# Adoni5/mappy-rs

Measured on AMD Instinct MI355X. Metric: aligned Mbases/sec, ONT reads vs GRCh38 map-ont, 1/2/4/8 MI355X, higher is better.
Workload: dtype u8/int32 (+f32 chaining gap cost, f64 RMQ priority)

## Files before the change

mappy-rs_amd/csrc/mm355_dp.hip:

```cpp
#include <hip/hip_runtime.h>
#include <stdio.h>
#include <string.h>
#include <vector>
#include <mutex>
#include <condition_variable>
#include <algorithm>
#include "mm355_pipeline.h"
#include "mm355_dp.h"
#include "mm355_dpdomain.h"

#define WAVE 64
#define KSW_NEG_INF (-0x40000000)

struct EzState { int32_t max, max_q, max_t, mqe, mqe_t, mte, mte_q, score, zdropped, reach_end; };

__device__ inline int8_t I8(int v) { return (int8_t)v; }

__device__ __forceinline__ bool apply_zdrop(EzState &ez, int32_t H, int r, int t, int zdrop, int e2)
{
	if (H > ez.max) {
		ez.max = H, ez.max_t = t, ez.max_q = r - t;
	} else if (t >= ez.max_t && r - t >= ez.max_q) {
		int tl = t - ez.max_t, ql = (r - t) - ez.max_q, l;
		l = tl > ql? tl - ql : ql - tl;
// ... 221 lines not shown
			if (r - st0 == qlen - 1 && Hst0 > ez.mqe) ez.mqe = Hst0, ez.mqe_t = st0;
			if (apply_zdrop(ez, max_H, r, max_t, zdrop, e2)) break;
			if (r == qlen + tlen - 2 && en0 == tlen - 1) ez.score = H[tlen - 1];
		} else {
			if (r > 0) {
				if (last_H0_t >= st0 && last_H0_t <= en0 && last_H0_t + 1 >= st0 && last_H0_t + 1 <= en0) {
					int32_t d0 = SB(S[last_H0_t], 1);
					int32_t d1 = SB(S[last_H0_t + 1], 0);
					if (d0 > d1) H0 += d0;
					else H0 += d1, ++last_H0_t;
				} else if (last_H0_t >= st0 && last_H0_t <= en0) {
					H0 += SB(S[last_H0_t], 1);
				} else {
					++last_H0_t, H0 += SB(S[last_H0_t], 0);
				}
			} else H0 = (int32_t)SB(S[0], 1) - qe, last_H0_t = 0;
			if ((flag & EZ_APPROX_DROP) && apply_zdrop(ez, H0, r, last_H0_t, zdrop, e2)) break;
			if (r == qlen + tlen - 2 && en0 == tlen - 1) ez.score = H0;
		}
		last_st = st, last_en = en;
		DP_SYNC();
	}
	if (lane == 0) {
		int i0 = -1, j0 = -1;
		if (!ez.zdropped && !(flag & EZ_EXTZ_ONLY)) { i0 = tlen - 1; j0 = qlen - 1; }
		else if (!ez.zdropped && (flag & EZ_EXTZ_ONLY) && ez.mqe + end_bonus > ez.max) { ez.reach_end = 1; i0 = ez.mqe_t; j0 = qlen - 1; }
		else if (ez.max_t >= 0 && ez.max_q >= 0) { i0 = ez.max_t; j0 = ez.max_q; }
		mm355_dpres_t o;
		o.max = ez.max; o.zdropped = ez.zdropped; o.max_q = ez.max_q; o.max_t = ez.max_t; o.mqe = ez.mqe; o.mqe_t = ez.mqe_t;
		o.mte = ez.mte; o.mte_q = ez.mte_q; o.score = ez.score; o.reach_end = ez.reach_end;
		o.n_cigar = i0;
		o.cigar_off = j0;
		res[jid] = o;
		if (cells) atomicAdd((cls_base >= 0? cells_ctr + DP_CTR_SPREAD * (2 * (cls_base + (T > 4096) + (T > 12288)) + (approx_max? 0 : 1)) : cells_ctr) + (blockIdx.x & (DP_CTR_SPREAD - 1)), cells);
	}
}

#include "mm355_dpreg.h"
#include "mm355_dpmw.h"
#include "mm355_dprow.h"
#include "mm355_dpband.h"

__global__ __launch_bounds__(WAVE) void k_ksw_backtrack(const DpJobDev *jobs, const int32_t *job_ids, int n_jobs, const uint8_t *pbase, const uint8_t *pbase2, uint32_t *cigbase,
                                                        mm355_dpres_t *res, uint32_t *dense, unsigned long long *dense_ctr)
{
	const int t = blockIdx.x * WAVE + threadIdx.x;
	if (t >= n_jobs) return;
	const int jid = job_ids[t];
	const DpJobDev jb = jobs[jid];
	mm355_dpres_t o = res[jid];
	const int i0 = o.n_cigar, j0 = (int)o.cigar_off;
	int n_cigar = 0;
	uint32_t *cigar = cigbase + jb.cig_off;
	const int qlen = jb.qlen, tlen = jb.tlen;
	if (qlen > 0 && tlen > 0 && !jb.skip && (i0 >= 0 || j0 >= 0)) {
		int w = jb.w;
		if (w < 0) w = tlen > qlen? tlen : qlen;
		int n_col_ = qlen < tlen? qlen : tlen;
		n_col_ = ((n_col_ < w + 1? n_col_ : w + 1) + 15) / 16 + 1;
		const int n_col = n_col_ * 16;
		const uint8_t *p = (jb.pad & 4? pbase2 : pbase) + jb.p_off;
		const int lay = jb.pad & 3, dlo = jb.dlo;
		const int row_stride = lay == 2? jb.bw : (tlen + 15) / 16 * 16 + 16;
		int i = i0, j = j0, state = 0;
		uint32_t run_op = 0, run_len = 0;
#define BT_PUSH(op, len) do { if (run_len && run_op == (uint32_t)(op)) run_len += (uint32_t)(len); else { if (run_len) cigar[n_cigar++] = run_len << 4 | run_op; run_op = (uint32_t)(op); run_len = (uint32_t)(len); } } while (0)
		while (i >= 0 && j >= 0) {
			int force_state = -1, rr = i + j;
			int st = 0, en = tlen - 1;
			if (st < rr - qlen + 1) st = rr - qlen + 1;
			if (en > rr) en = rr;
			if (st < (rr - w + 1) >> 1) st = (rr - w + 1) >> 1;
			if (en > (rr + w) >> 1) en = (rr + w) >> 1;
			st = st / 16 * 16, en = (en + 16) / 16 * 16 - 1;
			uint32_t tmp;
			if (i < st) force_state = 2;
			if (i > en) force_state = 1;
			tmp = force_state < 0? (lay == 1? p[row_cell_off(j, i, row_stride)] : lay == 2? p[row_cell_off(j, min(max(i - j - dlo, 0), row_stride - 1), row_stride)] : p[(size_t)rr * n_col + i - st]) : 0;
			if (state == 0) state = tmp & 7;
			else if (!(tmp >> (state + 2) & 1)) state = 0;
			if (state == 0) state = tmp & 7;
			if (force_state >= 0) state = force_state;
			if (state == 0) { BT_PUSH(0, 1); --i; --j; }
			else if (state == 1 || state == 3) { BT_PUSH(2, 1); --i; }
			else { BT_PUSH(1, 1); --j; }
		}
		if (i >= 0) BT_PUSH(2, i + 1);
		if (j >= 0) BT_PUSH(1, j + 1);
		if (run_len) cigar[n_cigar++] = run_len << 4 | run_op;
#undef BT_PUSH
	}
	long long dst;
	{
		const int lane = threadIdx.x & 63;
		unsigned int inc = (unsigned int)n_cigar;
		for (int d = 1; d < 64; d <<= 1) { const unsigned int u = __shfl_up(inc, d); if (lane >= d) inc += u; }
		const int last = 63 - __builtin_clzll(__ballot(1));
		unsigned long long base = 0;
		if (lane == last) base = atomicAdd(dense_ctr, (unsigned long long)inc);
		base = __shfl(base, last);
		dst = (long long)(base + inc - (unsigned int)n_cigar);
	}
	if (jb.flag & EZ_REV_CIGAR) for (int k = 0; k < n_cigar; ++k) dense[dst + k] = cigar[k];
	else for (int k = 0; k < n_cigar; ++k) dense[dst + k] = cigar[n_cigar - 1 - k];
	o.n_cigar = n_cigar; o.cigar_off = dst;
	res[jid] = o;
}

__global__ __launch_bounds__(256) void k_dp_gather(DevIndex ix, const DpGather *g, int n_jobs, const uint8_t *rq, uint8_t *qbuf, uint8_t *tbuf)
{
	const int j = blockIdx.x;
	if (j >= n_jobs) return;
	const DpGather gj = g[j];
	for (int i = threadIdx.x; i < gj.qlen; i += 256) {
		const int src = gj.rev? gj.qlen - 1 - i : i;
		qbuf[gj.qoff + i] = rq[gj.q_src + src];
	}
	const uint64_t base = ix.seq_off[gj.rid] + (uint64_t)gj.t_st;
	__shared__ uint32_t s_first, s_cnt;
	if (threadIdx.x == 0) { uint32_t f = 0, n = 0; if (ix.n_nr) ref_window(ix, base, base + (uint64_t)(gj.tlen > 0? gj.tlen : 0), f, n); s_first = f; s_cnt = n; }
	__syncthreads();
	const uint32_t first = s_first, cnt = s_cnt;
	for (int i = threadIdx.x; i < gj.tlen; i += 256) {
		const int src = gj.rev? gj.tlen - 1 - i : i;
		tbuf[gj.toff + i] = (uint8_t)ref_code(ix, first, cnt, base + (uint64_t)src);
	}
}

__global__ __launch_bounds__(256) void k_read_codes(DevBatch bt, uint8_t *rq)
{
	const int r = blockIdx.x;
	const int len = bt.rlen[r];
	const int64_t off = bt.roff[r];
	for (int i = threadIdx.x; i < len; i += 256) {
		const int c = mm_nt4(bt.seq[off + i]);
		rq[2 * off + i] = (uint8_t)c;
		rq[2 * off + len + (len - 1 - i)] = (uint8_t)(c < 4? 3 - c : 4);
	}
}

static const DpKnobs &dp_knobs()
{
	static const DpKnobs kn = [] {
		auto on = [](const char *name) { const char *e = getenv(name); return !(e && atoi(e) == 0); };
		DpKnobs k;
		k.use_row = on("MM355_DP_ROW"); k.use_rowl = on("MM355_DP_ROWL"); k.use_regw = on("MM355_DP_REGW"); k.regw8 = on("MM355_DP_REGW8");
		k.use_band = on("MM355_DP_BAND");
		if (const char *e = getenv("MM355_DP_BAND_THR")) k.band_thr = atof(e);
		if (const char *e = getenv("MM355_DP_BAND_THR_HALF")) k.band_thr_half = atof(e);
		if (const char *e = getenv("MM355_DP_BAND_FORCE")) k.band_force = atoi(e);
		return k;
	}();
	return kn;
}

size_t mm355_dp_matrix_bytes(const mm355_mapopt_t *mo, const DpConst &dc, int qlen, int tlen, int w_in, int flag)
{
	return mm355_dp_plan_budget(mm355_dp_plan(dc, dp_knobs(), mo->max_sw_mat, qlen, tlen, w_in, flag));
}

__global__ void k_dp_patch(DpJobDev *jobs, const int32_t *ids, const DpJobDev *nj, int n) { const int i = blockIdx.x * blockDim.x + threadIdx.x; if (i < n) jobs[ids[i]] = nj[i]; }

struct DpLaunchArgs {
	DpConst dc; const DpJobDev *jobs; const uint8_t *d_q, *d_t; uint8_t *bt; mm355_dpres_t *res;
	int32_t *d_off; uint32_t *cig; uint64_t *d_S; int32_t *d_H; uint32_t *dense; unsigned long long *d_dense;
	int32_t *d_fail;
	unsigned long long *d_gcells;
	size_t regw_seq;
	size_t n_band2_right;
};
typedef int (*DpLauncher)(const DpLaunchArgs &a, hipStream_t st, const int32_t *ids, unsigned n, unsigned long long *cells);

typedef void (*DpKernel)(DpConst, const DpJobDev*, const int32_t*, int, const uint8_t*, const uint8_t*, uint8_t*, mm355_dpres_t*, unsigned long long*);
template <DpKernel K, int NT = 64>
static int launch(const DpLaunchArgs &a, hipStream_t st, const int32_t *ids, unsigned n, unsigned long long *cells)
{
	hipLaunchKernelGGL(K, dim3(n), dim3(NT), 0, st, a.dc, a.jobs, ids, (int)n, a.d_q, a.d_t, a.bt, a.res, cells);
	return 0;
}
template <int CLS>
static int launch_lds(const DpLaunchArgs &a, hipStream_t st, const int32_t *ids, unsigned n, unsigned long long *)
{
	const int cap = DP_CLASS_CAP[CLS];
	(void)hipFuncSetAttribute((const void*)k_ksw_extd2<512>, hipFuncAttributeMaxDynamicSharedMemorySize, DP_CLASS_CAP[DP_N_CLASS - 2] * 12);
	hipLaunchKernelGGL(k_ksw_extd2<512>, dim3(n), dim3(512), (size_t)cap * 12, st, a.dc, a.jobs, ids, (int)n, a.d_q, a.d_t, a.bt, a.d_off, a.cig, a.d_S, a.d_H, a.res,
	                   cap, a.d_gcells, a.dense, a.d_dense, 4);
	return 0;
}
static int launch_regw(const DpLaunchArgs &a, hipStream_t st, const int32_t *ids, unsigned n, unsigned long long *cells)
{
	if (!dp_knobs().regw8) return launch<k_ksw_regw>(a, st, ids, n, cells);
	if (a.regw_seq + 64 > 32768 && hipFuncSetAttribute((const void*)k_ksw_regw8, hipFuncAttributeMaxDynamicSharedMemorySize, MW_SEQ_MAX + 64) != hipSuccess) return MM355_EHIP;
	hipLaunchKernelGGL(k_ksw_regw8, dim3(n), dim3(MW_THREADS), a.regw_seq + 64, st, a.dc, a.jobs, ids, (int)n, a.d_q, a.d_t, a.bt, a.res, cells);
	return 0;
}
template <int NS>
static int launch_band(const DpLaunchArgs &a, hipStream_t st, const int32_t *ids, unsigned n, unsigned long long *cells)
{
	hipLaunchKernelGGL(k_ksw_band<NS>, dim3(n), dim3(64), 0, st, a.dc, a.jobs, ids, (int)n, a.d_q, a.d_t, a.bt, a.res, cells, a.d_fail);
	return 0;
}
static int launch_band2(const DpLaunchArgs &a, hipStream_t st, const int32_t *ids, unsigned n, unsigned long long *cells)
{
	const unsigned nr = (unsigned)a.n_band2_right, nl = n - nr;
	if (nr) hipLaunchKernelGGL(k_ksw_band2, dim3((nr + 1) / 2), dim3(64), 0, st, a.dc, a.jobs, ids, (int)nr, a.d_q, a.d_t, a.bt, a.res, cells, a.d_fail);
	if (nl) hipLaunchKernelGGL(k_ksw_band2, dim3((nl + 1) / 2), dim3(64), 0, st, a.dc, a.jobs, ids + nr, (int)nl, a.d_q, a.d_t, a.bt, a.res, cells, a.d_fail);
	return 0;
}

struct DpUnit { int g0, g1; DpLauncher launch; int stream; bool in_turn, join_at_once; };
static const DpUnit DP_UNITS[] = {
	{ DP_G_LDS + 2, DP_G_ROW2,      launch_lds<5>,                       5, false, false },
// ... 24 lines not shown
	std::mutex m; std::condition_variable cv; int busy = 0;
	void lock(int cap) { std::unique_lock<std::mutex> lk(m); cv.wait(lk, [&] { return busy < cap; }); ++busy; }
	void unlock() { { std::lock_guard<std::mutex> lk(m); --busy; } cv.notify_one(); }
};
struct TurnGuard { Turn *t = 0; void lock(Turn *x, int cap) { x->lock(cap); t = x; } void unlock() { if (t) { t->unlock(); t = 0; } } ~TurnGuard() { unlock(); } };

static int group_begin(mm355_ctx *c, int g, hipStream_t gst)
{
	if (c->dp_ev[g] == 0) HIPCHK(hipEventCreateWithFlags(&c->dp_ev[g], hipEventDisableTiming));
	HIPCHK(hipStreamWaitEvent(gst, c->dp_up_ev, 0));
	if (c->dp_ev0[g] == 0) HIPCHK(hipEventCreate(&c->dp_ev0[g]));
	if (c->dp_ev1[g] == 0) HIPCHK(hipEventCreate(&c->dp_ev1[g]));
	HIPCHK(hipEventRecord(c->dp_ev0[g], gst));
	return 0;
}
static int group_end(mm355_ctx *c, int g, hipStream_t gst, bool join)
{
	HIPCHK(hipEventRecord(c->dp_ev1[g], gst));
	HIPCHK(hipEventRecord(c->dp_ev[g], gst));
	if (join) HIPCHK(hipStreamWaitEvent(c->st, c->dp_ev[g], 0));
	return 0;
}

int mm355_dp_run(mm355_ctx *c, const mm355_mapopt_t *mo, DpJobDev *jobs, size_t n, const uint8_t *d_q, const uint8_t *d_t, HBuf *arena,
                 const mm355_dpres_t **res_out, const uint32_t **cigar_out)
{
	*res_out = 0; *cigar_out = 0;
	if (n == 0) return 0;
	const DpConst dc = mm355_dp_const(mo);
	const DpKnobs &kn = dp_knobs();
	size_t p_tot = 0, cig_tot = 0, st_tot = 0, regw_seq = 0;
	std::vector<uint8_t> grp(n);
	size_t n_grp[DP_N_GROUP + 1] = {0};
	const int LB = 1024;
	std::vector<uint32_t> lcnt(LB + 1, 0);
	for (size_t i = 0; i < n; ++i) {
		DpJobDev &j = jobs[i];
		const DpPlan p = mm355_dp_plan(dc, kn, mo->max_sw_mat, j.qlen, j.tlen, j.w, j.flag);
		if (p.line) p_tot = (p_tot + 63) & ~(size_t)63;
		j.skip = p.skip; j.pad = p.pad; j.dlo = p.dlo; j.lmin = p.lmin; j.bw = p.bw; j.rsv = 0;
		j.p_off = (int64_t)p_tot; j.off_off = 0; j.cig_off = (int64_t)cig_tot; j.st_off = p.st_words? (int64_t)st_tot : 0;
		p_tot += p.bt_bytes; cig_tot += p.cig_words; st_tot += p.st_words;
		if (p.regw_lds > regw_seq) regw_seq = p.regw_lds;
		grp[i] = (uint8_t)p.group; ++n_grp[p.group];
		int lb = (j.qlen + j.tlen) >> 3; if (lb < 0) lb = 0; if (lb >= LB) lb = LB - 1;
		++lcnt[LB - 1 - lb];
	}
	if (const char *dump = getenv("MM355_DP_DUMP")) {
		static std::mutex dm; std::lock_guard<std::mutex> lk(dm);
		if (FILE *fp = fopen(dump, "ab")) { for (size_t i = 0; i < n; ++i) { int32_t v[4] = { jobs[i].qlen, jobs[i].tlen, jobs[i].w, jobs[i].flag }; fwrite(v, 4, 4, fp); } fclose(fp); }
	}
	if (c->h_ids.ensure((2 * n + 64) * 4)) return MM355_ENOMEM;
	int32_t *h_ids = (int32_t*)c->h_ids.p, *h_ord = h_ids + n + 8;
	size_t grp_off[DP_N_GROUP + 1], n_half_right = 0;
	{
		size_t acc = 0;
		for (int g = 0; g < DP_N_GROUP; ++g) { grp_off[g] = acc; acc += n_grp[g]; }
		grp_off[DP_N_GROUP] = acc;
		size_t cur[DP_N_GROUP];
		for (int g = 0; g < DP_N_GROUP; ++g) cur[g] = grp_off[g];
		uint32_t a2 = 0;
		for (int k = 0; k <= LB; ++k) { uint32_t t = lcnt[k]; lcnt[k] = a2; a2 += t; }
		for (size_t i = 0; i < n; ++i) {
			int lb = (jobs[i].qlen + jobs[i].tlen) >> 3; if (lb < 0) lb = 0; if (lb >= LB) lb = LB - 1;
			h_ord[lcnt[LB - 1 - lb]++] = (int32_t)i;
		}
		for (size_t k = 0; k < n; ++k) { const int32_t i = h_ord[k]; h_ids[cur[grp[i]]++] = i; }
		n_half_right = (size_t)(std::stable_partition(h_ids + grp_off[DP_G_BANDH], h_ids + grp_off[DP_G_BANDH] + n_grp[DP_G_BANDH], [&](int32_t i) { return (jobs[i].flag & EZ_RIGHT) != 0; }) - (h_ids + grp_off[DP_G_BANDH]));
	}
	auto unit_jobs = [&](const DpUnit &u) { return grp_off[u.g1] - grp_off[u.g0]; };
	if (c->dp_jobs.ensure(n * sizeof(DpJobDev)) || c->dp_res.ensure(n * sizeof(mm355_dpres_t)) || c->dp_bt.ensure(p_tot + 64, 4) ||
	    c->dp_work.ensure(16 * 4 + (2 * n + 32) * 4) || c->dp_cig.ensure((cig_tot + 16) * 4) || c->dp_dense.ensure((cig_tot + 16) * 4) ||
	    c->dp_H.ensure((st_tot + 16) * 12)) return MM355_ENOMEM;
	static std::vector<Turn> dp_turn((size_t)mm355_device_count());
	static const int turn_cap = [] { const char *e = getenv("MM355_DP_TURNS"); return e? atoi(e) : 1; }();
	const bool take_turns = turn_cap > 0;
	TurnGuard turn;
	HIPCHK(hipMemcpyAsync(c->dp_jobs.p, jobs, n * sizeof(DpJobDev), hipMemcpyHostToDevice, c->st));
	int32_t *d_off = c->dp_work.as<int32_t>();
	int32_t *d_ids = d_off + 16;
	uint64_t *d_S = c->dp_H.as<uint64_t>();
	unsigned long long *d_cells = c->counters.as<unsigned long long>() + 4, *d_dense = c->counters.as<unsigned long long>() + 5;
	bool redo_timed = false;
	HIPCHK(hipMemsetAsync(d_dense, 0, 8, c->st));
	unsigned long long *d_gcells = c->counters.as<unsigned long long>() + CTR_GCELLS_OFF;
	HIPCHK(hipMemsetAsync(d_cells, 0, 8, c->st));
	HIPCHK(hipMemsetAsync(d_gcells, 0, CTR_GCELLS_WORDS * 8, c->st));
	const size_t n_band = n_grp[DP_G_BAND1] + n_grp[DP_G_BAND2] + n_grp[DP_G_BAND4] + n_grp[DP_G_BANDH];
	if (c->dp_fail.ensure((2 * n_band + 64) * 4 + (n_band + 8) * sizeof(DpJobDev)) || c->h_fail.ensure((2 * n_band + 64) * 4 + (n_band + 8) * sizeof(DpJobDev))) return MM355_ENOMEM;
	int32_t *d_fail = c->dp_fail.as<int32_t>();
	if (n_band) HIPCHK(hipMemsetAsync(d_fail, 0, 4, c->st));
	HIPCHK(hipMemcpyAsync(d_ids, h_ids, (2 * n + 8) * 4, hipMemcpyHostToDevice, c->st));
	if (c->dp_up_ev == 0) HIPCHK(hipEventCreateWithFlags(&c->dp_up_ev, hipEventDisableTiming));
	HIPCHK(hipEventRecord(c->dp_up_ev, c->st));
	DpLaunchArgs la = { dc, c->dp_jobs.as<DpJobDev>(), d_q, d_t, c->dp_bt.as<uint8_t>(), c->dp_res.as<mm355_dpres_t>(), d_off, c->dp_cig.as<uint32_t>(), d_S, (int32_t*)(d_S + st_tot + 8),
	                    c->dp_dense.as<uint32_t>(), d_dense, d_fail, d_gcells, regw_seq, n_half_right };
	auto launch_units = [&](bool in_turn) -> int {
		for (const DpUnit &u : DP_UNITS) {
			if (u.in_turn != in_turn || unit_jobs(u) == 0) continue;
			hipStream_t gst; int rc;
			if ((rc = c->dp_stream(u.stream, &gst)) || (rc = group_begin(c, u.g0, gst))) return rc;
			if ((rc = u.launch(la, gst, d_ids + grp_off[u.g0], (unsigned)unit_jobs(u), d_gcells + DP_CTR_SPREAD * u.g0))) return rc;
			if ((rc = group_end(c, u.g0, gst, u.join_at_once))) return rc;
		}
		return 0;
	};
	if (int rc = launch_units(false)) return rc;
	if (take_turns) { HIPCHK(mm355_wait_stream(c->st)); turn.lock(&dp_turn[c->dev], turn_cap); }
	const double t_turn0 = mm355_now_ms();
	{
		EvTimer2 tm(c, &c->stats.ms_dp);
		if (int rc = launch_units(true)) return rc;
		if (n_band) {
			int32_t *h_fail = (int32_t*)c->h_fail.p;
			HIPCHK(hipMemcpyAsync(h_fail, d_fail, (1 + n_band) * 4, hipMemcpyDeviceToHost, c->st));
			HIPCHK(mm355_wait_stream(c->st));
			const size_t n_fail = (size_t)h_fail[0];
			c->stats.n_dp_band += (int64_t)n_band; c->stats.n_dp_band_redo += (int64_t)n_fail;
			if (n_fail) {
				std::sort(h_fail + 1, h_fail + 1 + n_fail);
				int32_t *h_rid = h_fail + 1 + n_band;
				DpJobDev *h_rj = (DpJobDev*)((char*)c->h_fail.p + (2 * n_band + 64) * 4);
				size_t p2 = 0, cnt[4] = {0, 0, 0, 0}, pos[4];
				for (size_t k = 0; k < n_fail; ++k) ++cnt[dp_redo_class(jobs[h_fail[1 + k]])];
				pos[0] = 0; pos[1] = cnt[0]; pos[2] = pos[1] + cnt[1]; pos[3] = pos[2] + cnt[2];
				for (size_t k = 0; k < n_fail; ++k) {
					DpJobDev &j = jobs[h_fail[1 + k]];
					j.pad = 1 | 4; j.p_off = (int64_t)p2; j.bw = 0;
					p2 += (row_matrix_bytes(j.qlen, (j.tlen + 15) / 16 * 16) + 63) & ~(size_t)63;
					h_rj[k] = j;
					h_rid[pos[dp_redo_class(j)]++] = h_fail[1 + k];
				}
				if (c->dp_bt2.ensure(p2 + 64, 4)) return MM355_ENOMEM;
				int32_t *d_rid = d_fail + 1 + n_band; DpJobDev *d_rj = (DpJobDev*)((char*)c->dp_fail.p + (2 * n_band + 64) * 4);
				HIPCHK(hipMemcpyAsync(d_fail + 1, h_fail + 1, n_fail * 4, hipMemcpyHostToDevice, c->st));
				HIPCHK(hipMemcpyAsync(d_rid, h_rid, n_fail * 4, hipMemcpyHostToDevice, c->st));
				HIPCHK(hipMemcpyAsync(d_rj, h_rj, n_fail * sizeof(DpJobDev), hipMemcpyHostToDevice, c->st));
				hipLaunchKernelGGL(k_dp_patch, dim3((unsigned)((n_fail + 255) / 256)), dim3(256), 0, c->st, c->dp_jobs.as<DpJobDev>(), d_fail + 1, d_rj, (int)n_fail);
				const int g = DP_G_REDO;
				if (c->dp_ev0[g] == 0) HIPCHK(hipEventCreate(&c->dp_ev0[g]));
				if (c->dp_ev1[g] == 0) HIPCHK(hipEventCreate(&c->dp_ev1[g]));
				HIPCHK(hipEventRecord(c->dp_ev0[g], c->st));
				DpLaunchArgs la2 = la; la2.bt = c->dp_bt2.as<uint8_t>();
				for (int k = 0; k < 4; ++k) {
					if (cnt[k]) (void)DP_REDO_LAUNCH[k](la2, c->st, d_rid, (unsigned)cnt[k], d_gcells + DP_CTR_SPREAD * g);
					d_rid += cnt[k];
				}
				HIPCHK(hipEventRecord(c->dp_ev1[g], c->st));
				redo_timed = true;
			}
		}
		if (take_turns) { const double tl1 = mm355_now_ms(); HIPCHK(mm355_wait_stream(c->st)); turn.unlock(); const double tl2 = mm355_now_ms(); mm355_trace_add(c, "dpk", t_turn0, tl2); mm355_trace_add(c, "dpk_launch", t_turn0, tl1); }
		for (const DpUnit &u : DP_UNITS) if (!u.join_at_once && unit_jobs(u)) HIPCHK(hipStreamWaitEvent(c->st, c->dp_ev[u.g0], 0));
		KtScope ks_bt(c, KT_DP_BACKTRACK, c->st);
		hipLaunchKernelGGL(k_ksw_backtrack, dim3((unsigned)((n + WAVE - 1) / WAVE)), dim3(WAVE), 0, c->st, c->dp_jobs.as<DpJobDev>(), d_ids + n + 8, (int)n,
		                   c->dp_bt.as<uint8_t>(), c->dp_bt2.as<uint8_t>(), c->dp_cig.as<uint32_t>(), c->dp_res.as<mm355_dpres_t>(), c->dp_dense.as<uint32_t>(), d_dense);
	}
	HIPCHK(hipGetLastError());
	if (c->h_res.ensure(n * sizeof(mm355_dpres_t) + 64 + CTR_GCELLS_WORDS * 8)) return MM355_ENOMEM;
	unsigned long long *ctr = (unsigned long long*)((char*)c->h_res.p + n * sizeof(mm355_dpres_t));
	HIPCHK(hipMemcpyAsync(ctr, d_cells, 16, hipMemcpyDeviceToHost, c->st));
	HIPCHK(hipMemcpyAsync(ctr + 2, d_gcells, CTR_GCELLS_WORDS * 8, hipMemcpyDeviceToHost, c->st));
	HIPCHK(hipMemcpyAsync(c->h_res.p, c->dp_res.p, n * sizeof(mm355_dpres_t), hipMemcpyDeviceToHost, c->st));
	HIPCHK(mm355_wait_stream(c->st));
	if (const char *dump = getenv("MM355_DP_DUMP_BT")) {
		std::vector<uint8_t> hb(p_tot + 64);
		if (hipMemcpy(hb.data(), c->dp_bt.p, p_tot, hipMemcpyDeviceToHost) == hipSuccess) if (FILE *fp = fopen(dump, "wb")) { fwrite(hb.data(), 1, p_tot, fp); fclose(fp); }
	}
	const size_t n_dense = (size_t)ctr[1];
	if (arena->ensure((n_dense + 16) * 4)) return MM355_ENOMEM;
	if (n_dense) HIPCHK(hipMemcpyAsync(arena->p, c->dp_dense.p, n_dense * 4, hipMemcpyDeviceToHost, c->st));
	HIPCHK(mm355_wait_stream(c->st));
	auto group_cells = [&](int g) { int64_t gc = 0; for (int k = 0; k < DP_CTR_SPREAD; ++k) gc += (int64_t)ctr[2 + DP_CTR_SPREAD * g + k]; return gc; };
	auto group_ms = [&](int g) { float ms = 0.f; if (hipEventElapsedTime(&ms, c->dp_ev0[g], c->dp_ev1[g]) == hipSuccess) c->stats.ms_dp_group[g] += ms; };
	int64_t tot = 0;
	for (const DpUnit &u : DP_UNITS) {
		if (unit_jobs(u) == 0) continue;
		group_ms(u.g0);
		for (int g = u.g0; g < u.g1; ++g) {
			if (n_grp[g] == 0) continue;
			const int64_t gc = group_cells(g);
			c->stats.dp_cells_group[g] += gc; ++c->stats.n_launch_group[g];
			tot += gc;
		}
	}
	if (redo_timed) {
		group_ms(DP_G_REDO);
		c->stats.dp_cells_group[DP_G_REDO] += group_cells(DP_G_REDO); ++c->stats.n_launch_group[DP_G_REDO];
	}
	c->stats.dp_cells += tot; c->stats.n_dp_jobs += (int64_t)n; ++c->stats.n_launch_dp;
	*res_out = (const mm355_dpres_t*)c->h_res.p; *cigar_out = (const uint32_t*)arena->p;
	return 0;
}

__device__ __forceinline__ uint32_t ex_target(const DevIndex &ix, const uint64_t o, uint32_t &nri)
{
	uint32_t c = ix.S2[o >> 4] >> ((o & 15) << 1) & 3u;
	while (nri < ix.n_nr && ix.nr[2 * nri + 1] <= o) ++nri;
	if (nri < ix.n_nr && ix.nr[2 * nri] <= o) c = 4;
	return c;
}

__global__ __launch_bounds__(WAVE) void k_extra(DevIndex ix, const uint8_t *rq, const Mm355ExtraJob *segs, int n_segs, const uint32_t *cig, Mm355ExtraScore sc,
                                                 char *cs, Mm355ExtraSegOut *out, int want)
{
	const int k = blockIdx.x * WAVE + threadIdx.x;
	if (k >= n_segs) return;
	const Mm355ExtraJob jb = segs[k];
	const uint8_t *q = rq + jb.q_src;
// ... 300 lines not shown
```

mappy-rs_amd/csrc/mm355_dprow.h:

```cpp
#pragma once
#include "mm355_dpplan.h"

__host__ __device__ __forceinline__ size_t row_cell_off(int q, int t, int tstride) { return (size_t)(q >> 2) * (size_t)(4 * tstride) + (size_t)(t >> 1) * 8 + (size_t)((q & 3) * 2 + (t & 1)); }

__device__ __forceinline__ uint32_t pk8w(int v) { const uint32_t h = (uint32_t)(uint16_t)(int16_t)v; return h | h << 16; }
__device__ __forceinline__ uint32_t pk_sign16(uint32_t a) { uint32_t r; asm("v_pk_ashrrev_i16 %0, 15, %1 op_sel_hi:[0,1]" : "=v"(r) : "v"(a)); return r; }
__device__ __forceinline__ uint32_t pk_rsubsat_s(uint32_t c, uint32_t a) { uint32_t r; asm("v_pk_sub_u16 %0, %1, %2 clamp" : "=v"(r) : "s"(c), "v"(a)); return r; }
__device__ __forceinline__ uint32_t pk_mad_vsv(uint32_t a, uint32_t b, uint32_t c) { uint32_t r; asm("v_pk_mad_u16 %0, %1, %2, %3" : "=v"(r) : "v"(a), "s"(b), "v"(c)); return r; }
__device__ __forceinline__ int32_t wave_incl_scan_max32(int32_t x)
{
	int32_t y;
	y = __builtin_amdgcn_update_dpp(INT32_MIN, x, 0x111, 0xf, 0xf, false); x = x > y? x : y;
	y = __builtin_amdgcn_update_dpp(INT32_MIN, x, 0x112, 0xf, 0xf, false); x = x > y? x : y;
	y = __builtin_amdgcn_update_dpp(INT32_MIN, x, 0x114, 0xf, 0xf, false); x = x > y? x : y;
	y = __builtin_amdgcn_update_dpp(INT32_MIN, x, 0x118, 0xf, 0xf, false); x = x > y? x : y;
	y = __builtin_amdgcn_update_dpp(INT32_MIN, x, 0x142, 0xa, 0xf, false); x = x > y? x : y;
	y = __builtin_amdgcn_update_dpp(INT32_MIN, x, 0x143, 0xc, 0xf, false); x = x > y? x : y;
	return x;
}

struct RowK {
	uint32_t qe1, e1, qe2, e2, q1, q2, mch, N, one, two, three, four, f8, f16, f32, f64;
	uint32_t q1p, q2p;
	int32_t q1i, q2i;
};

__device__ __forceinline__ int row_hb(int t, const DpConst &dc)
{
	if (t < 0) return 0;
	const int lt = dc.long_thres;
	int n1 = lt - 1 < t? lt - 1 : t; if (n1 < 0) n1 = 0;
	const int has = (lt >= 1 && lt <= t)? 1 : 0;
	const int n2 = t - n1 - has;
	return -(dc.q + dc.e) - n1 * dc.e + has * dc.long_diff - n2 * dc.e2;
}

__device__ __forceinline__ uint32_t pk2(int lo, int hi) { return (uint32_t)(uint16_t)(int16_t)lo | (uint32_t)(uint16_t)(int16_t)hi << 16; }
__device__ __forceinline__ uint32_t pk_max_swap(uint32_t a) { uint32_t r; asm("v_pk_max_i16 %0, %1, %1 op_sel:[0,1] op_sel_hi:[1,0]" : "=v"(r) : "v"(a)); return r; }

#define ROW_PKNEG 0x80008000u
__device__ __forceinline__ int32_t row_dbl(int v) { return (int32_t)((uint32_t)(v & 0xffff) * 0x10001u); }
__device__ __forceinline__ uint32_t row_scan(const uint32_t A, int32_t &C)
{
	const int32_t incl = wave_incl_scan_max32((int32_t)pk_max_swap(A));
	int32_t ex = __builtin_amdgcn_update_dpp(C, incl, 0x138, 0xf, 0xf, false);
	ex = ex > C? ex : C;
	const int32_t tot = __builtin_amdgcn_readlane(incl, 63);
	C = C > tot? C : tot;
	return pk_max((uint32_t)ex, __builtin_amdgcn_perm(A, ROW_PKNEG, 0x05040100));
}

template <bool RIGHT>
__device__ __forceinline__ void row_set(const RowK &K, const uint32_t dmis, const bool any_n, const uint32_t qc2, uint32_t &Hp, uint32_t &Fp, uint32_t &F2p,
                                        const uint32_t TQ, const uint32_t KE1, const uint32_t KE2, const uint32_t KQ1, const uint32_t KQ2, uint32_t &carry_h, int32_t &C1, int32_t &C2, const bool odd, uint32_t &accw)
{
	const uint32_t sh = (uint32_t)__builtin_amdgcn_update_dpp((int)carry_h, (int)Hp, 0x138, 0xf, 0xf, false);
// ... 240 lines not shown
```

Measured before the change: 1444.

## Add wave-per-job backtrack kernel with LDS windows for long alignments

```diff
diff --git a/mappy-rs_amd/csrc/mm355_btwalk.h b/mappy-rs_amd/csrc/mm355_btwalk.h
--- /dev/null
+++ b/mappy-rs_amd/csrc/mm355_btwalk.h
@@ -0,0 +1,220 @@
+#pragma once
+#include <stdint.h>
+#include <stddef.h>
+#if defined(__HIPCC__)
+#include <hip/hip_runtime.h>
+#define BT_HD __host__ __device__ __forceinline__
+#else
+#define BT_HD inline
+#endif
+
+BT_HD size_t row_cell_off(int q, int t, int tstride) { return (size_t)(q >> 2) * (size_t)(4 * tstride) + (size_t)(t >> 1) * 8 + (size_t)((q & 3) * 2 + (t & 1)); }
+
+struct BtGeom {
+	int qlen, tlen, w;
+	int n_col;
+	int lay, dlo;
+	int row_stride;
+};
+
+BT_HD BtGeom bt_geom(int qlen, int tlen, int w, int pad, int dlo, int bw)
+{
+	BtGeom g;
+	g.qlen = qlen; g.tlen = tlen;
+	g.w = w < 0? (tlen > qlen? tlen : qlen) : w;
+	int n_col_ = qlen < tlen? qlen : tlen;
+	n_col_ = ((n_col_ < g.w + 1? n_col_ : g.w + 1) + 15) / 16 + 1;
+	g.n_col = n_col_ * 16;
+	g.lay = pad & 3; g.dlo = dlo;
+	g.row_stride = g.lay == 2? bw : (tlen + 15) / 16 * 16 + 16;
+	return g;
+}
+
+BT_HD void bt_diag_range(const BtGeom &g, int rr, int &st, int &en)
+{
+	st = 0, en = g.tlen - 1;
+	if (st < rr - g.qlen + 1) st = rr - g.qlen + 1;
+	if (en > rr) en = rr;
+	if (st < (rr - g.w + 1) >> 1) st = (rr - g.w + 1) >> 1;
+	if (en > (rr + g.w) >> 1) en = (rr + g.w) >> 1;
+	st = st / 16 * 16, en = (en + 16) / 16 * 16 - 1;
+}
+
+BT_HD int bt_force(int i, int st, int en) { return i > en? 1 : i < st? 2 : -1; }
+
+BT_HD int64_t bt_cell_off(const BtGeom &g, int i, int j, int st)
+{
+	if (g.lay == 1) return (int64_t)row_cell_off(j, i, g.row_stride);
+	if (g.lay == 2) { int c = i - j - g.dlo; c = c < 0? 0 : c; c = c > g.row_stride - 1? g.row_stride - 1 : c; return (int64_t)row_cell_off(j, c, g.row_stride); }
+	return (int64_t)(i + j) * g.n_col + i - st;
+}
+
+BT_HD int64_t bt_row_base(const BtGeom &g, int row) { return g.lay? (int64_t)row * (4 * (int64_t)g.row_stride) : (int64_t)row * g.n_col; }
+template <int LAY> BT_HD int bt_cell_x(const BtGeom &g, int i, int j, int st)
+{
+	if (LAY == 0) return i - st;
+	int c = i;
+	if (LAY == 2) { c = i - j - g.dlo; c = c < 0? 0 : c; c = c > g.row_stride - 1? g.row_stride - 1 : c; }
+	return (c >> 1) * 8 + (j & 3) * 2 + (c & 1);
+}
+
+struct BtWalk { int i, j, state; uint32_t run_op, run_len; int n_cigar; };
+
+BT_HD BtWalk bt_start(int i0, int j0) { BtWalk k; k.i = i0; k.j = j0; k.state = 0; k.run_op = k.run_len = 0; k.n_cigar = 0; return k; }
+
+BT_HD void bt_push(BtWalk &k, uint32_t *cigar, uint32_t op, uint32_t len)
+{
+	if (k.run_op != op) { if (k.run_len) cigar[k.n_cigar++] = k.run_len << 4 | k.run_op; k.run_op = op; k.run_len = 0; }
+	k.run_len += len;
+}
+
+BT_HD void bt_step(BtWalk &k, uint32_t *cigar, uint32_t tmp, int force_state)
+{
+	int state = k.state;
+	if (state == 0) state = tmp & 7;
+	else if (!(tmp >> (state + 2) & 1)) state = 0;
+	if (state == 0) state = tmp & 7;
+	if (force_state >= 0) state = force_state;
+	if (state == 0) { bt_push(k, cigar, 0, 1); --k.i; --k.j; }
+	else if (state == 1 || state == 3) { bt_push(k, cigar, 2, 1); --k.i; }
+	else { bt_push(k, cigar, 1, 1); --k.j; }
+	k.state = state;
+}
+
+BT_HD int bt_finish(BtWalk &k, uint32_t *cigar)
+{
+	if (k.i >= 0) bt_push(k, cigar, 2, (uint32_t)(k.i + 1));
+	if (k.j >= 0) bt_push(k, cigar, 1, (uint32_t)(k.j + 1));
+	if (k.run_len) cigar[k.n_cigar++] = k.run_len << 4 | k.run_op;
+	k.run_len = 0;
+	return k.n_cigar;
+}
+
+BT_HD int bt_walk_literal(const BtGeom &g, const uint8_t *p, int i0, int j0, uint32_t *cigar)
+{
+	BtWalk k = bt_start(i0, j0);
+	while (k.i >= 0 && k.j >= 0) {
+		int st, en;
+		bt_diag_range(g, k.i + k.j, st, en);
+		const int force_state = bt_force(k.i, st, en);
+		const uint32_t tmp = force_state < 0? p[bt_cell_off(g, k.i, k.j, st)] : 0;
+		bt_step(k, cigar, tmp, force_state);
+	}
+	return bt_finish(k, cigar);
+}
+
+template <int R> struct BtWin {
+	static constexpr int SW0 = (R + 15) / 16 * 16 + 16;
+	static constexpr int SW12 = 4 * R + 64;
+	static constexpr int NS12 = R / 4 + 1;
+	static constexpr int N_META = R > NS12? R : NS12;
+	static constexpr int BYTES = R * SW0 > NS12 * SW12? R * SW0 : NS12 * SW12;
+	static_assert(R % 4 == 0 && R >= 4, "a window is whole tile rows");
+};
+
+struct BtStrip { int64_t base; int32_t rel, len; };
+struct BtDiag { int32_t st, en; };
+
+template <int R> BT_HD int bt_n_strips(const BtGeom &g) { return g.lay? BtWin<R>::NS12 : R; }
+template <int R> BT_HD int bt_strip_width(const BtGeom &g) { return g.lay? BtWin<R>::SW12 : BtWin<R>::SW0; }
+BT_HD int bt_strip_row(const BtGeom &g, int i0, int j0, int s) { return g.lay? (j0 >> 2) - s : i0 + j0 - s; }
+
+template <int R> BT_HD void bt_strip_range(const BtGeom &g, int i0, int j0, int s, int narrow, int64_t &lo, int64_t &hi)
+{
+	lo = 0; hi = -1;
+	if (g.lay == 0) {
+		const int rr = i0 + j0 - s;
+		if (rr < 0) return;
+		int st, en;
+		bt_diag_range(g, rr, st, en);
+		int a = i0 - s + narrow, b = i0;
+		if (a < st) a = st;
+		if (a < 0) a = 0;
+		if (b > en) b = en;
+		if (b > rr) b = rr;
+		if (b > st + g.n_col - 1) b = st + g.n_col - 1;
+		if (a > b) return;
+		lo = (int64_t)rr * g.n_col + a - st; hi = (int64_t)rr * g.n_col + b - st;
+		return;
+	}
+	const int G = (j0 >> 2) - s;
+	if (G < 0) return;
+	const int q_hi = 4 * G + 3 < j0? 4 * G + 3 : j0, q_lo = 4 * G > j0 - (R - 1)? 4 * G : j0 - (R - 1);
+	if (q_lo > q_hi) return;
+	int a = i0 - (R - 1) + (j0 - q_hi) + narrow, b = i0;
+	if (g.lay == 2) {
+		a = a - q_hi - g.dlo; b = b - q_lo - g.dlo;
+		if (a > g.row_stride - 1) a = g.row_stride - 1;
+		if (b > g.row_stride - 1) b = g.row_stride - 1;
+		if (b < 0) b = 0;
+	} else if (b > g.tlen - 1) b = g.tlen - 1;
+	if (a < 0) a = 0;
+	if (a > b) return;
+	const int64_t row = (int64_t)G * (4 * (int64_t)g.row_stride);
+	lo = row + (int64_t)(a >> 1) * 8; hi = row + (int64_t)(b >> 1) * 8 + 7;
+}
+
+BT_HD BtStrip bt_strip_stage(int64_t lo, int64_t hi, int64_t must, int align, int width, int64_t row_base)
+{
+	BtStrip m; m.base = 0; m.rel = 0; m.len = 0;
+	if (must >= 0) { if (hi < lo) lo = hi = must; if (must < lo) lo = must; if (must > hi) hi = must; }
+	if (hi < lo) return m;
+	m.base = ((lo + align) & ~(int64_t)15) - align;
+	int64_t len = ((hi - m.base) / 16 + 1) * 16;
+	if (len > width) { len = width; if (must >= 0 && must - m.base >= len) { m.base = ((must + align) & ~(int64_t)15) - align; len = 16; } }
+	m.rel = (int32_t)(m.base - row_base); m.len = (int32_t)len;
+	return m;
+}
+
+template <int R> BT_HD BtStrip bt_strip(const BtGeom &g, int i0, int j0, int s, int narrow, int align)
+{
+	int64_t lo, hi, must = -1;
+	bt_strip_range<R>(g, i0, j0, s, narrow, lo, hi);
+	if (s == 0) { int st, en; bt_diag_range(g, i0 + j0, st, en); if (bt_force(i0, st, en) < 0) must = bt_cell_off(g, i0, j0, st); }
+	return bt_strip_stage(lo, hi, must, align, bt_strip_width<R>(g), bt_row_base(g, bt_strip_row(g, i0, j0, s)));
+}
+
+BT_HD BtDiag bt_diag(const BtGeom &g, int i0, int j0, int k) { BtDiag d; bt_diag_range(g, i0 + j0 - k, d.st, d.en); return d; }
+
+template <int R, int LAY, class Stage> BT_HD int bt_probe(const BtGeom &g, int i, int j, int i0, int j0, const Stage &sg)
+{
+	if (i < 0 || j < 0) return -1;
+	const int dk = i0 + j0 - (i + j);
+	if (dk >= R) return -1;
+	const int s = LAY? (j0 >> 2) - (j >> 2) : dk;
+	BtDiag de; BtStrip m;
+	sg.meta_any(dk, s, de, m);
+	if (bt_force(i, de.st, de.en) >= 0) return -1;
+	const uint32_t d = (uint32_t)(bt_cell_x<LAY>(g, i, j, de.st) - m.rel);
+	if (d >= (uint32_t)m.len) return -1;
+	return (int)sg.byte_any(s * (LAY? BtWin<R>::SW12 : BtWin<R>::SW0) + (int)d);
+}
+
+template <int R, int LAY, class Stage> BT_HD bool bt_walk_window(const BtGeom &g, BtWalk &k, uint32_t *cigar, int i0, int j0, const Stage &sg)
+{
+	const int rr0 = i0 + j0, width = LAY? BtWin<R>::SW12 : BtWin<R>::SW0;
+	while (k.i >= 0 && k.j >= 0) {
+		if (k.state == 0) {
+			const int n = sg.template match_run<R, LAY>(g, k.i, k.j, i0, j0);
+			if (n > 0) { bt_push(k, cigar, 0, (uint32_t)n); k.i -= n; k.j -= n; continue; }
+		}
+		const int dk = rr0 - (k.i + k.j);
+		if (dk >= R) return false;
+		const int s = LAY? (j0 >> 2) - (k.j >> 2) : dk;
+		BtDiag de; BtStrip m;
+		sg.meta(dk, s, de, m);
+		const int force_state = bt_force(k.i, de.st, de.en);
+		uint32_t tmp = 0;
+		if (force_state < 0) {
+			const uint32_t d = (uint32_t)(bt_cell_x<LAY>(g, k.i, k.j, de.st) - m.rel);
+			if (d >= (uint32_t)m.len) return false;
+			tmp = sg.byte(s * width + (int)d);
+		}
+		bt_step(k, cigar, tmp, force_state);
+	}
+	return true;
+}
+template <int R, class Stage> BT_HD bool bt_walk_window(const BtGeom &g, BtWalk &k, uint32_t *cigar, int i0, int j0, const Stage &sg)
+{
+	return g.lay == 0? bt_walk_window<R, 0>(g, k, cigar, i0, j0, sg) : g.lay == 1? bt_walk_window<R, 1>(g, k, cigar, i0, j0, sg) : bt_walk_window<R, 2>(g, k, cigar, i0, j0, sg);
+}
diff --git a/mappy-rs_amd/csrc/mm355_dp.hip b/mappy-rs_amd/csrc/mm355_dp.hip
--- a/mappy-rs_amd/csrc/mm355_dp.hip
+++ b/mappy-rs_amd/csrc/mm355_dp.hip
@@ -297,44 +297,8 @@
 	const int i0 = o.n_cigar, j0 = (int)o.cigar_off;
 	int n_cigar = 0;
 	uint32_t *cigar = cigbase + jb.cig_off;
-	const int qlen = jb.qlen, tlen = jb.tlen;
-	if (qlen > 0 && tlen > 0 && !jb.skip && (i0 >= 0 || j0 >= 0)) {
-		int w = jb.w;
-		if (w < 0) w = tlen > qlen? tlen : qlen;
-		int n_col_ = qlen < tlen? qlen : tlen;
-		n_col_ = ((n_col_ < w + 1? n_col_ : w + 1) + 15) / 16 + 1;
-		const int n_col = n_col_ * 16;
-		const uint8_t *p = (jb.pad & 4? pbase2 : pbase) + jb.p_off;
-		const int lay = jb.pad & 3, dlo = jb.dlo;
-		const int row_stride = lay == 2? jb.bw : (tlen + 15) / 16 * 16 + 16;
-		int i = i0, j = j0, state = 0;
-		uint32_t run_op = 0, run_len = 0;
-#define BT_PUSH(op, len) do { if (run_len && run_op == (uint32_t)(op)) run_len += (uint32_t)(len); else { if (run_len) cigar[n_cigar++] = run_len << 4 | run_op; run_op = (uint32_t)(op); run_len = (uint32_t)(len); } } while (0)
-		while (i >= 0 && j >= 0) {
-			int force_state = -1, rr = i + j;
-			int st = 0, en = tlen - 1;
-			if (st < rr - qlen + 1) st = rr - qlen + 1;
-			if (en > rr) en = rr;
-			if (st < (rr - w + 1) >> 1) st = (rr - w + 1) >> 1;
-			if (en > (rr + w) >> 1) en = (rr + w) >> 1;
-			st = st / 16 * 16, en = (en + 16) / 16 * 16 - 1;
-			uint32_t tmp;
-			if (i < st) force_state = 2;
-			if (i > en) force_state = 1;
-			tmp = force_state < 0? (lay == 1? p[row_cell_off(j, i, row_stride)] : lay == 2? p[row_cell_off(j, min(max(i - j - dlo, 0), row_stride - 1), row_stride)] : p[(size_t)rr * n_col + i - st]) : 0;
-			if (state == 0) state = tmp & 7;
-			else if (!(tmp >> (state + 2) & 1)) state = 0;
-			if (state == 0) state = tmp & 7;
-			if (force_state >= 0) state = force_state;
-			if (state == 0) { BT_PUSH(0, 1); --i; --j; }
-			else if (state == 1 || state == 3) { BT_PUSH(2, 1); --i; }
-			else { BT_PUSH(1, 1); --j; }
-		}
-		if (i >= 0) BT_PUSH(2, i + 1);
-		if (j >= 0) BT_PUSH(1, j + 1);
-		if (run_len) cigar[n_cigar++] = run_len << 4 | run_op;
-#undef BT_PUSH
-	}
+	if (jb.qlen > 0 && jb.tlen > 0 && !jb.skip && (i0 >= 0 || j0 >= 0))
+		n_cigar = bt_walk_literal(bt_geom(jb.qlen, jb.tlen, jb.w, jb.pad, jb.dlo, jb.bw), (jb.pad & 4? pbase2 : pbase) + jb.p_off, i0, j0, cigar);
 	long long dst;
 	{
 		const int lane = threadIdx.x & 63;
@@ -350,6 +314,100 @@
 	else for (int k = 0; k < n_cigar; ++k) dense[dst + k] = cigar[n_cigar - 1 - k];
 	o.n_cigar = n_cigar; o.cigar_off = dst;
 	res[jid] = o;
+}
+
+#define BT_R 64
+__device__ __forceinline__ int bt_uni(int v) { return __builtin_amdgcn_readfirstlane(v); }
+struct BtLdsStage {
+	const uint8_t *win; const BtStrip *mt; const BtDiag *dg;
+	__device__ __forceinline__ void meta(int k, int s, BtDiag &d, BtStrip &m) const
+	{
+		const BtDiag vd = dg[k]; const int rel = mt[s].rel, len = mt[s].len;
+		asm volatile("" :: "v"(vd.st), "v"(vd.en), "v"(rel), "v"(len));
+		d.st = bt_uni(vd.st); d.en = bt_uni(vd.en); m.base = 0; m.rel = bt_uni(rel); m.len = bt_uni(len);
+	}
+	__device__ __forceinline__ uint32_t byte(int x) const { return (uint32_t)bt_uni((int)win[x]); }
+	__device__ __forceinline__ void meta_any(int k, int s, BtDiag &d, BtStrip &m) const { d = dg[k]; m.base = 0; m.rel = mt[s].rel; m.len = mt[s].len; }
+	__device__ __forceinline__ uint32_t byte_any(int x) const { return win[x]; }
+	template <int R, int LAY> __device__ __forceinline__ int match_run(const BtGeom &g, int i, int j, int i0, int j0) const
+	{
+		const int l = (int)threadIdx.x, b = bt_probe<R, LAY>(g, i - l, j - l, i0, j0, *this);
+		const unsigned long long stop = __ballot(b < 0 || (b & 7));
+		return stop? __builtin_ctzll(stop) : WAVE;
+	}
+};
+
+struct BtPieces { uint4 v0, v1, v2, v3, v4; int dst, n; };
+__device__ __forceinline__ BtPieces bt_fetch(const BtGeom &g, const uint8_t *p, int align, int wi, int wj, int u, BtStrip *s_meta)
+{
+	static_assert(BtWin<BT_R>::SW0 == 5 * 16 && BtWin<BT_R>::SW12 == 4 * 5 * 16, "a strip is one unit or four");
+	const int sh = g.lay? 2 : 0, s = u >> sh, piece = (u & ((1 << sh) - 1)) * 5;
+	BtPieces q; q.dst = 0; q.n = 0;
+	q.v0 = q.v1 = q.v2 = q.v3 = q.v4 = make_uint4(0, 0, 0, 0);
+	if (s < bt_n_strips<BT_R>(g)) {
+		const BtStrip m = bt_strip<BT_R>(g, wi, wj, s, 0, align);
+		if (piece == 0) s_meta[s] = m;
+		const uint4 *src = (const uint4*)(p + m.base) + piece;
+		q.n = m.len / 16 - piece; q.dst = s * bt_strip_width<BT_R>(g) + piece * 16;
+		if (q.n > 0) q.v0 = src[0];
+		if (q.n > 1) q.v1 = src[1];
+		if (q.n > 2) q.v2 = src[2];
+		if (q.n > 3) q.v3 = src[3];
+		if (q.n > 4) q.v4 = src[4];
+	}
+	return q;
+}
+__device__ __forceinline__ void bt_put(uint8_t *s_win, const BtPieces &q)
+{
+	uint4 *d = (uint4*)(s_win + q.dst);
+	if (q.n > 0) d[0] = q.v0;
+	if (q.n > 1) d[1] = q.v1;
+	if (q.n > 2) d[2] = q.v2;
+	if (q.n > 3) d[3] = q.v3;
+	if (q.n > 4) d[4] = q.v4;
+}
+
+__global__ __launch_bounds__(WAVE) void k_ksw_backtrack_wave(const DpJobDev *jobs, const int32_t *job_ids, int n_jobs, const uint8_t *pbase, const uint8_t *pbase2, uint32_t *cigbase,
+                                                             mm355_dpres_t *res, uint32_t *dense, unsigned long long *dense_ctr)
+{
+	typedef BtWin<BT_R> Win;
+	static_assert(Win::NS12 * 4 <= 2 * WAVE && BT_R <= WAVE, "two units per lane cover a window");
+	__shared__ __attribute__((aligned(16))) uint8_t s_win[Win::BYTES];
+	__shared__ BtStrip s_meta[Win::N_META];
+	__shared__ BtDiag s_diag[BT_R];
+	if ((int)blockIdx.x >= n_jobs) return;
+	const int lane = threadIdx.x;
+	const int jid = bt_uni(job_ids[blockIdx.x]);
+	const DpJobDev &jb = jobs[jid];
+	const int i0 = bt_uni(res[jid].n_cigar), j0 = bt_uni((int)res[jid].cigar_off);
+	const int qlen = bt_uni(jb.qlen), tlen = bt_uni(jb.tlen), pad = bt_uni(jb.pad), rev = bt_uni(jb.flag & EZ_REV_CIGAR);
+	int n_cigar = 0;
+	uint32_t *cigar = cigbase + jb.cig_off;
+	if (qlen > 0 && tlen > 0 && !bt_uni(jb.skip) && (i0 >= 0 || j0 >= 0)) {
+		const BtGeom g = bt_geom(qlen, tlen, bt_uni(jb.w), pad, bt_uni(jb.dlo), bt_uni(jb.bw));
+		const uint8_t *p = (pad & 4? pbase2 : pbase) + jb.p_off;
+		const int align = (int)((uintptr_t)p & 15);
+		const BtLdsStage sg = { s_win, s_meta, s_diag };
+		BtWalk k = bt_start(i0, j0);
+		bool done = k.i < 0 || k.j < 0;
+		while (!done) {
+			const int wi = k.i, wj = k.j;
+			const BtPieces q0 = bt_fetch(g, p, align, wi, wj, lane, s_meta), q1 = bt_fetch(g, p, align, wi, wj, lane + WAVE, s_meta);
+			if (lane < BT_R) s_diag[lane] = bt_diag(g, wi, wj, lane);
+			bt_put(s_win, q0); bt_put(s_win, q1);
+			__builtin_amdgcn_s_waitcnt(0x0f70);
+			__syncthreads();
+			done = bt_walk_window<BT_R>(g, k, cigar, wi, wj, sg);
+			__syncthreads();
+		}
+		n_cigar = bt_finish(k, cigar);
+	}
+	unsigned long long base = 0;
+	if (lane == 0) base = atomicAdd(dense_ctr, (unsigned long long)n_cigar);
+	const long long dst = (long long)__shfl(base, 0);
+	if (rev) for (int c = lane; c < n_cigar; c += WAVE) dense[dst + c] = cigar[c];
+	else for (int c = lane; c < n_cigar; c += WAVE) dense[dst + c] = cigar[n_cigar - 1 - c];
+	if (lane == 0) { res[jid].n_cigar = n_cigar; res[jid].cigar_off = dst; }
 }
 
 __global__ __launch_bounds__(256) void k_dp_gather(DevIndex ix, const DpGather *g, int n_jobs, const uint8_t *rq, uint8_t *qbuf, uint8_t *tbuf)
@@ -403,6 +461,9 @@
 {
 	return mm355_dp_plan_budget(mm355_dp_plan(dc, dp_knobs(), mo->max_sw_mat, qlen, tlen, w_in, flag));
 }
+
+#define BT_WAVE_MIN 1024
+static int bt_wave_min() { const char *e = getenv("MM355_BT_WAVE_MIN"); return e? atoi(e) : BT_WAVE_MIN; }
 
 __global__ void k_dp_patch(DpJobDev *jobs, const int32_t *ids, const DpJobDev *nj, int n) { const int i = blockIdx.x * blockDim.x + threadIdx.x; if (i < n) jobs[ids[i]] = nj[i]; }
 
@@ -533,7 +594,7 @@
 	}
 	if (c->h_ids.ensure((2 * n + 64) * 4)) return MM355_ENOMEM;
 	int32_t *h_ids = (int32_t*)c->h_ids.p, *h_ord = h_ids + n + 8;
-	size_t grp_off[DP_N_GROUP + 1], n_half_right = 0;
+	size_t grp_off[DP_N_GROUP + 1], n_half_right = 0, n_long = 0;
 	{
 		size_t acc = 0;
 		for (int g = 0; g < DP_N_GROUP; ++g) { grp_off[g] = acc; acc += n_grp[g]; }
@@ -546,6 +607,8 @@
 			int lb = (jobs[i].qlen + jobs[i].tlen) >> 3; if (lb < 0) lb = 0; if (lb >= LB) lb = LB - 1;
 			h_ord[lcnt[LB - 1 - lb]++] = (int32_t)i;
 		}
+		const int lb_long = (bt_wave_min() + 7) >> 3;
+		n_long = lb_long >= LB? 0 : lb_long <= 0? n : (size_t)lcnt[LB - 1 - lb_long];
 		for (size_t k = 0; k < n; ++k) { const int32_t i = h_ord[k]; h_ids[cur[grp[i]]++] = i; }
 		n_half_right = (size_t)(std::stable_partition(h_ids + grp_off[DP_G_BANDH], h_ids + grp_off[DP_G_BANDH] + n_grp[DP_G_BANDH], [&](int32_t i) { return (jobs[i].flag & EZ_RIGHT) != 0; }) - (h_ids + grp_off[DP_G_BANDH]));
 	}
@@ -634,8 +697,10 @@
 		if (take_turns) { const double tl1 = mm355_now_ms(); HIPCHK(mm355_wait_stream(c->st)); turn.unlock(); const double tl2 = mm355_now_ms(); mm355_trace_add(c, "dpk", t_turn0, tl2); mm355_trace_add(c, "dpk_launch", t_turn0, tl1); }
 		for (const DpUnit &u : DP_UNITS) if (!u.join_at_once && unit_jobs(u)) HIPCHK(hipStreamWaitEvent(c->st, c->dp_ev[u.g0], 0));
 		KtScope ks_bt(c, KT_DP_BACKTRACK, c->st);
-		hipLaunchKernelGGL(k_ksw_backtrack, dim3((unsigned)((n + WAVE - 1) / WAVE)), dim3(WAVE), 0, c->st, c->dp_jobs.as<DpJobDev>(), d_ids + n + 8, (int)n,
-		                   c->dp_bt.as<uint8_t>(), c->dp_bt2.as<uint8_t>(), c->dp_cig.as<uint32_t>(), c->dp_res.as<mm355_dpres_t>(), c->dp_dense.as<uint32_t>(), d_dense);
+		if (n_long) hipLaunchKernelGGL(k_ksw_backtrack_wave, dim3((unsigned)n_long), dim3(WAVE), 0, c->st, c->dp_jobs.as<DpJobDev>(), d_ids + n + 8, (int)n_long,
+		                               c->dp_bt.as<uint8_t>(), c->dp_bt2.as<uint8_t>(), c->dp_cig.as<uint32_t>(), c->dp_res.as<mm355_dpres_t>(), c->dp_dense.as<uint32_t>(), d_dense);
+		if (n > n_long) hipLaunchKernelGGL(k_ksw_backtrack, dim3((unsigned)((n - n_long + WAVE - 1) / WAVE)), dim3(WAVE), 0, c->st, c->dp_jobs.as<DpJobDev>(), d_ids + n + 8 + n_long, (int)(n - n_long),
+		                                   c->dp_bt.as<uint8_t>(), c->dp_bt2.as<uint8_t>(), c->dp_cig.as<uint32_t>(), c->dp_res.as<mm355_dpres_t>(), c->dp_dense.as<uint32_t>(), d_dense);
 	}
 	HIPCHK(hipGetLastError());
 	if (c->h_res.ensure(n * sizeof(mm355_dpres_t) + 64 + CTR_GCELLS_WORDS * 8)) return MM355_ENOMEM;
diff --git a/mappy-rs_amd/csrc/mm355_dprow.h b/mappy-rs_amd/csrc/mm355_dprow.h
--- a/mappy-rs_amd/csrc/mm355_dprow.h
+++ b/mappy-rs_amd/csrc/mm355_dprow.h
@@ -1,7 +1,7 @@
 #pragma once
 #include "mm355_dpplan.h"
 
-__host__ __device__ __forceinline__ size_t row_cell_off(int q, int t, int tstride) { return (size_t)(q >> 2) * (size_t)(4 * tstride) + (size_t)(t >> 1) * 8 + (size_t)((q & 3) * 2 + (t & 1)); }
+#include "mm355_btwalk.h"
 
 __device__ __forceinline__ uint32_t pk8w(int v) { const uint32_t h = (uint32_t)(uint16_t)(int16_t)v; return h | h << 16; }
 __device__ __forceinline__ uint32_t pk_sign16(uint32_t a) { uint32_t r; asm("v_pk_ashrrev_i16 %0, 15, %1 op_sel_hi:[0,1]" : "=v"(r) : "v"(a)); return r; }
```

Result: slower. 1407 (-2.6%).
